# Skylarking/MARL

Hardware: AMD Instinct MI355X
Metric: env_steps_per_sec (higher is better)
Workload: dtype f32 (bf16x6 split products, fp32 accumulate)

## Files before the change

include/marl_hip.h:

```cpp
#ifndef MARL_HIP_H
#define MARL_HIP_H
#include <stddef.h>
#ifdef __cplusplus
extern "C" {
#endif

typedef struct {
  const float* p0; long ld0; int k0;
  const float* p1; long ld1; int k1;
  const int* idx; int nhot; int hot_w;
  int nid;
  const float* m0; long ldm0;
  long rpe0, bs0, off0;
  long rpei, bsi, offi;
  const int* emap0;
} marl_src_t;

typedef struct {
  int groups;
  long gs_x0, gs_x1, gs_w, gs_b, gs_y, gs_m0;
} marl_group_t;

typedef struct {
  const float *fc1_w, *fc1_b;
// ... 86 lines not shown
int marl_qmix_wide_fwd(const marl_qmix_weights_t* w, const marl_src_t* s, const float* q, float* q_tot, float* ws,
                       size_t ws_bytes, long rows, int N, int S, int E, int flags, void* stream);
int marl_qmix_wide_bwd(const marl_qmix_weights_t* w, const marl_src_t* s, const float* q, const float* dq_tot, float* dq,
                       const marl_qmix_weights_t* grads, float* ws, size_t ws_bytes, long rows, int N, int S, int E,
                       int flags, void* stream);
int marl_qmix_wide_loss_bwd(const marl_qmix_weights_t* w, const marl_src_t* s, const float* q, const float* q_tot_tgt,
                            const float* r, const float* term, const float* padded, float gamma, float* q_tot, float* dq,
                            const marl_qmix_weights_t* grads, float* loss2, float* ws, size_t ws_bytes, long rows,
                            int N, int S, int E, int flags, void* stream);

typedef struct {
  const float *w1, *b1;
  const float *w2, *b2;
  const float *w3, *b3;
  long gs_w1, gs_b1, gs_w2, gs_b2, gs_w3, gs_b3;
} marl_mlp3_weights_t;
int marl_mlp3_supported(const marl_src_t* x, int K1, int H1, int H2, int N3, int groups);
int marl_mlp3_fwd(const marl_mlp3_weights_t* w, const marl_src_t* x, float* Y, long ldy, long gs_y,
                  long M, int K1, int N3, int groups, void* stream);
size_t marl_mlp3_bwd_workspace(long M, int K1, int N3, int groups);
int marl_mlp3_bwd(const marl_mlp3_weights_t* w, const marl_src_t* x, const float* dY, long lddy, long gs_dy,
                  const marl_mlp3_weights_t* grads, float* ws, size_t ws_bytes, long M, int K1, int N3,
                  int groups, void* stream);
size_t marl_mlp3_save_floats(long M, int three, int groups);
int marl_mlp3_needs_kept(const marl_src_t* x, int K1, int N3);
int marl_mlp3_fwd_save(const marl_mlp3_weights_t* w, const marl_src_t* x, float* Y, long ldy, long gs_y,
                       float* hsave, size_t hsave_floats, long M, int K1, int N3, int groups, void* stream);
int marl_mlp3_bwd_saved(const marl_mlp3_weights_t* w, const marl_src_t* x, const float* dY, long lddy, long gs_dy,
                        const marl_mlp3_weights_t* grads, float* ws, size_t ws_bytes, const float* hsave,
                        size_t hsave_floats, long M, int K1, int N3, int groups, void* stream);

int marl_agent_unroll_x6_supported(int B, int T, int N, int O, int A, int last_action, int reuse_network);
int marl_agent_unroll_x6_plain_r6(int B, int T, int N, int O, int A, int last_action, int reuse_network, int cu_budget);
int marl_agent_unroll_fwd_x6(const marl_agent_weights_t* w, const float* obs, long obs_bs, int obs_t0,
                             const int* ufed, long u_bs, int u_t0, const int* ep_len, const int* ep_map,
                             const float* h0, float* q, float* hs, float* h_last, float* saved, int B, int T, int N,
                             int O, int A, int last_action, int reuse_network, int cu_budget, float* gi_out,
                             const float* gi_in, void* stream);

int marl_agent_unroll_bwd_x6_supported(int B, int T, int N, int A, int sparse_dq);
size_t marl_agent_bwd_x6_workspace(int B, int N, int A);
int marl_agent_unroll_bwd_x6(const marl_agent_weights_t* w, const int* dq_idx, const float* dq_val, const int* dq_idx2,
                             const float* dq_val2, int dq_gdiv, const float* dhs, const float* saved, float* dxp, float* dh0,
                             const marl_agent_grads_t* g, float* ws, size_t ws_bytes, int B, int T, int N, int A, void* stream);

int marl_mlp3_x6_supported(const marl_src_t* x, int K1, int H1, int H2, int N3, int groups);
int marl_mlp3_x6_fwd_save(const marl_mlp3_weights_t* w, const marl_src_t* x, float* Y, long ldy, long gs_y,
                          float* hsave, size_t hsave_floats, long M, int K1, int N3, int groups, void* stream);
int marl_mlp3_x6_bwd_saved(const marl_mlp3_weights_t* w, const marl_src_t* x, const float* dY, long lddy, long gs_dy,
                           const marl_mlp3_weights_t* grads, float* ws, size_t ws_bytes, const float* hsave,
                           size_t hsave_floats, long M, int K1, int N3, int groups, void* stream);

typedef struct {
  const float *enc0_w, *enc0_b;
  const float *enc2_w, *enc2_b;
  const float* q0_w; long q0_ld; int q0_s;
  const float *q2_w, *q2_b;
  const float *q4_w, *q4_b;
} marl_qtran_weights_t;
int marl_qtran_supported(int N, int A, int AE);
int marl_qtran_head_fwd(const marl_qtran_weights_t* w, const float* hidden, const int* u, const float* sp, float* out,
                        float* s1, float* e2, float* y1, float* y2, long BT, int N, int A, int AE, void* stream);
int marl_qtran_head_fwd2(const marl_qtran_weights_t* w, const float* hidden, const int* u, const int* u2, const float* sp,
                         float* out, float* out2, float* s1, float* e2, float* y1, float* y2, long BT, int N, int A, int AE,
                         void* stream);
size_t marl_qtran_bwd_workspace(long BT, int AE);
// ... 143 lines not shown
```

marl_amd/_lib.py:

```python
from __future__ import annotations

import ctypes as C
import os

_HERE = os.path.dirname(os.path.abspath(__file__))
LIB_PATH = os.environ.get("MARL_HIP_LIB") or os.path.join(_HERE, "libmarl_hip.so")

c_float_p = C.c_void_p
c_int_p = C.c_void_p


class MarlSrc(C.Structure):
    _fields_ = [("p0", C.c_void_p), ("ld0", C.c_long), ("k0", C.c_int),
                ("p1", C.c_void_p), ("ld1", C.c_long), ("k1", C.c_int),
                ("idx", C.c_void_p), ("nhot", C.c_int), ("hot_w", C.c_int),
                ("nid", C.c_int),
                ("m0", C.c_void_p), ("ldm0", C.c_long),
                ("rpe0", C.c_long), ("bs0", C.c_long), ("off0", C.c_long),
                ("rpei", C.c_long), ("bsi", C.c_long), ("offi", C.c_long),
                ("emap0", C.c_void_p)]


class MarlGroup(C.Structure):
    _fields_ = [("groups", C.c_int), ("gs_x0", C.c_long), ("gs_x1", C.c_long), ("gs_w", C.c_long),
# ... 38 lines not shown
                                          "k_w", "k_b", "q_w", "q_b")]


class MarlAgentGrads(C.Structure):
    _fields_ = [("w_ih", C.c_void_p), ("w_hh", C.c_void_p), ("b_ih", C.c_void_p), ("b_hh", C.c_void_p),
                ("fc2_w", C.c_void_p), ("fc2_b", C.c_void_p)]


class MarlAgentWeights(C.Structure):
    _fields_ = [("fc1_w", C.c_void_p), ("fc1_b", C.c_void_p), ("w_ih", C.c_void_p), ("w_hh", C.c_void_p),
                ("b_ih", C.c_void_p), ("b_hh", C.c_void_p), ("fc2_w", C.c_void_p), ("fc2_b", C.c_void_p),
                ("H", C.c_int)]


P, I, L, F, U, SZ, D = C.c_void_p, C.c_int, C.c_long, C.c_float, C.c_uint, C.c_size_t, C.c_double
SRC, GRP, AW = C.POINTER(MarlSrc), C.POINTER(MarlGroup), C.POINTER(MarlAgentWeights)
AG = C.POINTER(MarlAgentGrads)
QW = C.POINTER(MarlQmixWeights)
M3 = C.POINTER(MarlMlp3Weights)
QT = C.POINTER(MarlQtranWeights)
RW = C.POINTER(MarlRtwWeights)
WW, WG = C.POINTER(MarlWorldWeights), C.POINTER(MarlWorldGrads)
MW, MG = C.POINTER(MarlMaicWeights), C.POINTER(MarlMaicGrads)

SIGNATURES = {
    "marl_linear": (I, [SRC, P, L, I, P, P, L, I, I, I, I, F, GRP, P]),
    "marl_linear_wgrad": (I, [P, L, P, L, SRC, P, L, P, I, I, I, I, GRP, P, SZ, P]),
    "marl_linear_wgrad_workspace": (SZ, [I, I, I, I]),
    "marl_wgrad_slabs": (I, [I]),
    "marl_agent_unroll_fwd": (I, [AW, P, L, I, P, L, I, P, P, P, P, P, P, P, I, I, I, I, I, I, I, I, P, P, P]),
    "marl_agent_unroll_reuse_supported": (I, [I, I, I, I, I, I]),
    "marl_agent_unroll_x6_supported": (I, [I, I, I, I, I, I, I]),
    "marl_agent_unroll_x6_plain_r6": (I, [I, I, I, I, I, I, I, I]),
    "marl_agent_unroll_fwd_x6": (I, [AW, P, L, I, P, L, I, P, P, P, P, P, P, P, I, I, I, I, I, I, I, I, P, P, P]),
    "marl_agent_bwd_workspace": (SZ, [I, I, I]),
    "marl_agent_unroll_bwd_x6_supported": (I, [I, I, I, I, I]),
    "marl_agent_bwd_x6_workspace": (SZ, [I, I, I]),
    "marl_agent_unroll_bwd_x6": (I, [AW, P, P, P, P, I, P, P, P, P, AG, P, SZ, I, I, I, I, P]),
    "marl_agent_unroll_bwd": (I, [AW, P, P, P, P, P, I, P, P, P, P, P, AG, P, SZ, I, I, I, I, P]),
    "marl_replay_gather": (I, [P, I, I, I, I] + [P] * 17 + [P]),
    "marl_q_gather": (I, [P, P, P, F, P, L, I, P]),
    "marl_q_masked_max": (I, [P, P, F, P, P, L, I, P]),
    "marl_q_double_select": (I, [P, P, P, F, P, P, L, I, P]),
    "marl_q_scatter": (I, [P, P, P, P, P, L, I, I, P]),
    "marl_vec_add": (I, [P, P, P, L, P]),
    "marl_agent_sum": (I, [P, L, P, L, L, I, I, P]),
    "marl_agent_bcast": (I, [P, L, P, L, L, I, I, I, P]),
    "marl_qmix_mix_fwd": (I, [P, L, P, P, P, P, P, L, I, I, P]),
    "marl_qmix_mix_bwd": (I, [P, L, P, P, P, P, P, P, L, I, I, P]),
    "marl_qmix_tail_fwd": (I, [SRC, L, I, P, L, P, P, L, P, P, L, I, I, P]),
    "marl_qmix_fused_supported": (I, [I, I, I]),
    "marl_qmix_fused_workspace": (SZ, [L, I, I]),
    "marl_qmix_fused_fwd": (I, [QW, SRC, P, P, L, I, I, I, P]),
    "marl_qmix_fused_bwd": (I, [QW, SRC, P, P, P, QW, P, SZ, L, I, I, I, P]),
    "marl_qmix_fused_loss_bwd": (I, [QW, SRC, P, P, P, P, P, F, P, P, QW, P, P, SZ, L, I, I, I, P]),
    "marl_qmix_fused_fwd_x6": (I, [QW, SRC, P, P, L, I, I, I, P]),
    "marl_qmix_fused_bwd_x6": (I, [QW, SRC, P, P, P, QW, P, SZ, L, I, I, I, P]),
    "marl_qmix_fused_loss_bwd_x6": (I, [QW, SRC, P, P, P, P, P, F, P, P, QW, P, P, SZ, L, I, I, I, P]),
    "marl_qmix_wide_supported": (I, [I, I, I]),
    "marl_qmix_wide_workspace": (SZ, [L, I, I, I]),
    "marl_qmix_wide_fwd_kernel": (C.c_char_p, [L, I, I, I]),
    "marl_qmix_wide_fwd": (I, [QW, SRC, P, P, P, SZ, L, I, I, I, I, P]),
    "marl_qmix_wide_bwd": (I, [QW, SRC, P, P, P, QW, P, SZ, L, I, I, I, I, P]),
    "marl_qmix_wide_loss_bwd": (I, [QW, SRC, P, P, P, P, P, F, P, P, QW, P, P, SZ, L, I, I, I, I, P]),
    "marl_mlp3_supported": (I, [SRC, I, I, I, I, I]),
    "marl_mlp3_fwd": (I, [M3, SRC, P, L, L, L, I, I, I, P]),
# ... 89 lines not shown
```

marl_amd/csrc/agent_x6.hip:

```cpp
#include "x6.h"
#include <cstdlib>
#include "../../include/marl_hip.h"

int marl_agent_x6p_tiles(int B, int T, int N, int O, int A, int last_action, int reuse_network, int cu_budget);
int marl_agent_x6p_launch(const marl_agent_weights_t* w, const float* obs, long obs_bs, int obs_t0, const int* ufed, long u_bs, int u_t0,
                          const int* ep_len, const int* ep_map, const float* h0, float* q, float* h_last, int B, int T, int N, int O, int A,
                          int last_action, int reuse_network, int tpw, void* stream);

namespace {

constexpr int H = 64;
constexpr int XNT = 512;
constexpr int HP = 72;
constexpr int NLD = 4;

struct X6Args {
  const float *W1, *b1, *Wih, *Whh, *bih, *bhh, *W2, *b2;
  const float* obs; long obs_bs; int obs_t0;
  const int* ufed; long u_bs; int u_t0;
  const int* ep_len; const int* ep_map;
  const float* h0;
  float *q, *hs, *h_last;
  float* saved;
  float* gi_out;
  const float* gi_in;
  int B, T, N, O, A, I, KI;
  int has_act, has_id, RT;
  int n_full;
  long R;
};

__device__ __forceinline__ f32x4 relu4x(const f32x4& v) { return (f32x4){fmaxf(v[0], 0.f), fmaxf(v[1], 0.f), fmaxf(v[2], 0.f), fmaxf(v[3], 0.f)}; }
__device__ __forceinline__ long sv_off(long tile_t, int planes, int plane, int c, int lane) {
  return ((tile_t * planes + plane) * 4 + c) * 256 + lane * 4;
}

template <int RTC, bool SAVE, bool XS, bool GIO = false, int NK1 = 3, int AC = 1>
__global__ __launch_bounds__(XNT, 2) void agent_fwd_x6_kernel(X6Args a) {
  static_assert(!(SAVE && XS) && (SAVE || !GIO), "XS: no saving; GIO: the saving pass also stores its input-side gate sums");
  extern __shared__ __attribute__((aligned(16))) char smem[];
// ... 384 lines not shown
        }
      }
      if (!FC2I && t > 0 && s < RTW) fc2(par, t - 1, s);
      if (NGR && t + 1 < a.T) nin(par ^ 1, t + 1);
      ST_MARK(2);
      if (ALLP) {
        if (par) commit(0, pu_lds0); else commit(1, pu_lds1);
        issue(t + 4 < a.T ? t + 4 : Tm1);
      }
      WG_BARRIER();
      ST_MARK(3);
    }
    if (!FC2I && s < RTW) fc2(a.T & 1, a.T - 1, s);
    ST_DUMP(4);
  }
}

}

extern "C" int marl_agent_unroll_x6_supported(int B, int T, int N, int O, int A, int last_action, int reuse_network) {
  const int I = O + (last_action ? A : 0) + (reuse_network ? N : 0);
  if (A < 1 || O < 8 || (O & 7) || I > 224 || T < 4 || B < 1) return 0;
  if (A > (I > 160 ? 32 : 16)) return 0;
  if (16 * (O / 4) > 3 * 256) return 0;
  if ((double)B * T * N * H * 4.0 >= 4294967296.0) return 0;
  return 1;
}

extern "C" int marl_agent_unroll_x6_plain_r6(int B, int T, int N, int O, int A, int last_action, int reuse_network, int cu_budget) {
  return marl_agent_unroll_x6_supported(B, T, N, O, A, last_action, reuse_network) &&
         marl_agent_x6p_tiles(B, T, N, O, A, last_action, reuse_network, cu_budget) ? 1 : 0;
}

extern "C" int marl_agent_unroll_fwd_x6(const marl_agent_weights_t* w, const float* obs, long obs_bs, int obs_t0,
                                        const int* ufed, long u_bs, int u_t0, const int* ep_len, const int* ep_map,
                                        const float* h0, float* q, float* hs, float* h_last, float* saved, int B, int T, int N,
                                        int O, int A, int last_action, int reuse_network, int cu_budget, float* gi_out,
                                        const float* gi_in, void* stream) {
  if (B <= 0 || T <= 0) return 0;
  if (w->H != H || cu_budget < 0 || cu_budget > 256 || !marl_agent_unroll_x6_supported(B, T, N, O, A, last_action, reuse_network))
    return (int)hipErrorInvalidValue;
  if (saved && gi_in) return (int)hipErrorInvalidValue;
  if (!saved && !gi_in && !hs && !(reinterpret_cast<uintptr_t>(h0) & 15) && !(reinterpret_cast<uintptr_t>(h_last) & 15)) {
    const int tpw = marl_agent_x6p_tiles(B, T, N, O, A, last_action, reuse_network, cu_budget);
    if (tpw) return marl_agent_x6p_launch(w, obs, obs_bs, obs_t0, ufed, u_bs, u_t0, ep_len, ep_map, h0, q, h_last, B, T, N, O, A, last_action,
                                          reuse_network, tpw, stream);
  }
  if ((reinterpret_cast<uintptr_t>(obs) & 15) || (h0 && (reinterpret_cast<uintptr_t>(h0) & 3)) || (saved && (reinterpret_cast<uintptr_t>(saved) & 15)) ||
      (gi_out && (reinterpret_cast<uintptr_t>(gi_out) & 15)) || (gi_in && (reinterpret_cast<uintptr_t>(gi_in) & 15)))
    return (int)hipErrorInvalidValue;
  if (cu_budget == 0) cu_budget = 256;
  X6Args a;
  a.W1 = w->fc1_w; a.b1 = w->fc1_b; a.Wih = w->w_ih; a.Whh = w->w_hh; a.bih = w->b_ih; a.bhh = w->b_hh; a.W2 = w->fc2_w; a.b2 = w->fc2_b;
  a.obs = obs; a.obs_bs = obs_bs; a.obs_t0 = obs_t0; a.ufed = ufed; a.u_bs = u_bs; a.u_t0 = u_t0; a.ep_len = ep_len; a.ep_map = ep_map;
  a.h0 = h0; a.q = q; a.hs = hs; a.h_last = h_last; a.saved = saved; a.gi_out = saved ? gi_out : nullptr; a.gi_in = gi_in;
  a.B = B; a.T = T; a.N = N; a.O = O; a.A = A;
  a.has_act = last_action ? 1 : 0; a.has_id = reuse_network ? 1 : 0;
  a.I = O + (last_action ? A : 0) + (reuse_network ? N : 0);
  a.KI = (a.I + 31) / 32 * 32;
  a.R = (long)B * N;
  const long tiles = (a.R + 15) / 16;
  const int wide = a.KI > 160 ? 2 : a.KI > 96 ? 1 : 0;
  const int rt = tiles > cu_budget && !wide ? 2 : 1;
  if (rt * 16 * (O / 4) > 3 * 256) return (int)hipErrorInvalidValue;
  a.RT = rt;
  long n_wg = (tiles + rt - 1) / rt;
  a.n_full = (int)n_wg;
  if (rt == 2) {
    const long k = (tiles + 2 * cu_budget - 1) / (2 * cu_budget), rem = tiles - 2L * cu_budget * (k - 1);
    if (rem <= cu_budget) { a.n_full = (int)(cu_budget * (k - 1)); n_wg = a.n_full + rem; }
  }
  const int rows = rt * 16, IP = a.KI + 8;
  const size_t lds = (size_t)2 * 3 * rows * IP * 2 + (size_t)4 * 3 * rows * HP * 2 + (size_t)2 * rt * 4 * 3 * 1024 + (size_t)rows * (2 * 8 + 4 * 4) +
                     (((size_t)T * 4 + 15) & ~(size_t)15) + (wide == 2 ? (size_t)4 * 2 * 3 * 1024 : 0);
  if (lds > 160 * 1024) return (int)hipErrorInvalidValue;
  const void* fn;
#define X6_PICKF(SAVE_, XS_, GIO_) (wide == 2 ? (const void*)agent_fwd_x6_kernel<1, SAVE_, XS_, GIO_, 7, 2>                         \
                                    : wide == 1 ? (const void*)agent_fwd_x6_kernel<1, SAVE_, XS_, GIO_, 5, 1>                       \
                                    : rt == 2 ? (const void*)agent_fwd_x6_kernel<2, SAVE_, XS_, GIO_, 3, 1> : (const void*)agent_fwd_x6_kernel<1, SAVE_, XS_, GIO_, 3, 1>)
// ... 17 lines not shown
```

marl_amd/csrc/agent_x6p.hip:

```cpp
#include "x6.h"
#include "../../include/marl_hip.h"

namespace {

constexpr int H = 64;
constexpr int PNT = 512;
constexpr int HP = 72;
constexpr int NPF = 7;

struct PX6Args {
  const float *W1, *b1, *Wih, *Whh, *bih, *bhh, *W2, *b2;
  const float* obs; long obs_bs; int obs_t0;
  const int* ufed; long u_bs; int u_t0;
  const int* ep_len; const int* ep_map;
  const float* h0;
  float *q, *h_last;
  int B, T, N, O, A, I, KI;
  int has_act, has_id;
  long R;
};

template <int RTC>
__global__ __launch_bounds__(PNT, 2) void agent_fwd_x6p_kernel(PX6Args a) {
  extern __shared__ __attribute__((aligned(16))) char smem[];
  const int tid = threadIdx.x, lane = tid & 63, wave = __builtin_amdgcn_readfirstlane(tid >> 6);
  const int team = wave >> 2, s = wave & 3;
  const int q = lane >> 4, m = lane & 15, u4 = 16 * s + 4 * q;
  constexpr int rows = 16 * RTC;
  const int T = a.T, N = a.N, O = a.O, A = a.A;
  const int IP = a.KI + 8;
  const int IN_E = 3 * rows * IP, XP_E = 3 * rows * HP;
  short* In0 = reinterpret_cast<short*>(smem);
  short* Xp0 = In0 + IN_E;
  short* Hp0 = Xp0 + XP_E;
  float* W1a = reinterpret_cast<float*>(Hp0 + 2 * XP_E);
  unsigned* rowobs = reinterpret_cast<unsigned*>(W1a + (A + 1) * H);
  unsigned* rowu = rowobs + rows;
  int* rowidx = reinterpret_cast<int*>(rowu + rows);
  int* rowlen = rowidx + rows;
  i32x4* W2f = reinterpret_cast<i32x4*>(rowlen + rows);
  auto hpp = [&](int b) { return Hp0 + b * XP_E; };

  const long row0 = (long)blockIdx.x * rows;
  for (int r = tid; r < rows; r += PNT) {
    long rho = row0 + r;
    if (rho > a.R - 1) rho = a.R - 1;
    const long b = rho / N;
    const int n = (int)(rho % N);
    rowidx[r] = (int)(b * T * N + n);
    rowobs[r] = (unsigned)((((a.ep_map ? (long)a.ep_map[b] : b) * a.obs_bs + n) * O) * 4);
    rowu[r] = (unsigned)((b * a.u_bs + n) * 4);
    rowlen[r] = a.ep_len ? a.ep_len[b] : 0x7fffffff;
// ... 245 lines not shown
    };
    issue(0);
    ufetch(0);
    commit(0);
    WG_BARRIER();
    fc1();
    xput(0);
    issue(1); ufetch(1);
    WG_BARRIER();
    commit(1);
    issue(2);
    WG_BARRIER();
    ST_DECL(4);
    for (int t = 0; t < T; ++t) {
      if (t + 1 < T) fc1();
      if (t >= 1) fc2(t & 1, t - 1, true);
      else landed();
      ST_MARK(0);
      WG_BARRIER();
      ST_MARK(1);
      if (t + 1 < T) xput(t + 1);
      commit(t + 2);
      issue(t + 3);
      ufetch(t + 2);
      ST_MARK(2);
      WG_BARRIER();
      ST_MARK(3);
    }
    ST_DUMP(4);
    fc2(T & 1, T - 1, false);
  }
}

static size_t px6_lds(int rtc, int KI, int A) {
  const size_t rows = 16 * (size_t)rtc, IP = KI + 8;
  return 3 * rows * IP * 2 + 3 * 3 * rows * HP * 2 + (size_t)(A + 1) * H * 4 + rows * (4 + 4 + 4 + 4) + (rtc >= 5 ? (size_t)2 * 3 * 4 * A * 16 : 0);
}

}

ST_DEFINE_SETTER(marl_debug_stamps_agent_x6p)

__attribute__((visibility("hidden"))) int marl_agent_x6p_tiles(int B, int T, int N, int O, int A, int last_action, int reuse_network, int cu_budget) {
  if (!marl_switches()->unroll_r6) return 0;
  const int I = O + (last_action ? A : 0) + (reuse_network ? N : 0);
  if (I > 96 || A < 1 || A > 16 || O < 8 || (O & 3) || T < 2 || B < 1) return 0;
  if (cu_budget != 0 && cu_budget != 256) return 0;
  const long tiles = ((long)B * N + 15) / 16;
  if (tiles <= 512) return 0;
  if ((long)16 * 5 * (O / 4) > 256L * NPF) return 0;
  if (T > 32000) return 0;
  if ((double)B * T * N * H * 4.0 >= 4294967296.0) return 0;
  int tpw = (int)((tiles + 255) / 256);
  if (tpw > 5) {
    const long rounds = (tiles + 256 * 5 - 1) / (256 * 5);
    tpw = (int)((tiles + 256 * rounds - 1) / (256 * rounds));
    if (tpw > 5) tpw = 5;
  }
  if (tpw < 3) tpw = 3;
  return px6_lds(tpw, (I + 31) / 32 * 32, A) <= 160 * 1024 ? tpw : 0;
}

__attribute__((visibility("hidden"))) int marl_agent_x6p_launch(const marl_agent_weights_t* w, const float* obs, long obs_bs, int obs_t0,
                                                                 const int* ufed, long u_bs, int u_t0, const int* ep_len, const int* ep_map,
                                                                 const float* h0, float* q, float* h_last, int B, int T, int N, int O, int A,
                                                                 int last_action, int reuse_network, int tpw, void* stream) {
  if ((reinterpret_cast<uintptr_t>(obs) & 15) || (h0 && (reinterpret_cast<uintptr_t>(h0) & 15)) || (h_last && (reinterpret_cast<uintptr_t>(h_last) & 15)))
    return (int)hipErrorInvalidValue;
  PX6Args a;
  a.W1 = w->fc1_w; a.b1 = w->fc1_b; a.Wih = w->w_ih; a.Whh = w->w_hh; a.bih = w->b_ih; a.bhh = w->b_hh; a.W2 = w->fc2_w; a.b2 = w->fc2_b;
  a.obs = obs; a.obs_bs = obs_bs; a.obs_t0 = obs_t0; a.ufed = ufed; a.u_bs = u_bs; a.u_t0 = u_t0; a.ep_len = ep_len; a.ep_map = ep_map;
  a.h0 = h0; a.q = q; a.h_last = h_last;
  a.B = B; a.T = T; a.N = N; a.O = O; a.A = A;
  a.has_act = last_action ? 1 : 0; a.has_id = reuse_network ? 1 : 0;
  a.I = O + (last_action ? A : 0) + (reuse_network ? N : 0);
  a.KI = (a.I + 31) / 32 * 32;
  a.R = (long)B * N;
  const long tiles = (a.R + 15) / 16;
  const size_t lds = px6_lds(tpw, a.KI, A);
  const void* fn = tpw == 3 ? (const void*)agent_fwd_x6p_kernel<3> : tpw == 4 ? (const void*)agent_fwd_x6p_kernel<4> : (const void*)agent_fwd_x6p_kernel<5>;
  hipError_t e = hipFuncSetAttribute(fn, hipFuncAttributeMaxDynamicSharedMemorySize, (int)lds);
  if (e != hipSuccess) return (int)e;
  dim3 grid((unsigned)((tiles + tpw - 1) / tpw)), block(PNT);
  void* kargs[] = {(void*)&a};
  e = hipLaunchKernel(fn, grid, block, kargs, lds, (hipStream_t)stream);
  if (e != hipSuccess) return (int)e;
  MARL_CHECK_LAUNCH();
  return 0;
}
```

marl_amd/ops.py:

```python
from __future__ import annotations

import ctypes as C

import torch

from . import _lib
from ._lib import (MarlSrc, MarlGroup, MarlAgentWeights, MarlAgentGrads, MarlQmixWeights, MarlMlp3Weights,
                   MarlQtranWeights, MarlRtwWeights, MarlWorldWeights, MarlWorldGrads, MarlMaicWeights, MarlMaicGrads, check)


def _p(t):
    return None if t is None else C.c_void_p(t.data_ptr())


def _stream():
    return C.c_void_p(torch.cuda.current_stream().cuda_stream)


def _f32(t):
    assert t.dtype == torch.float32 and t.is_cuda, "expected a CUDA float32 tensor"
    return t


def _i32(t):
# ... 105 lines not shown
    w = MarlAgentWeights()
    w.fc1_w, w.fc1_b = params["fc1.weight"].data_ptr(), params["fc1.bias"].data_ptr()
    w.w_ih, w.w_hh = params["rnn.weight_ih"].data_ptr(), params["rnn.weight_hh"].data_ptr()
    w.b_ih, w.b_hh = params["rnn.bias_ih"].data_ptr(), params["rnn.bias_hh"].data_ptr()
    w.fc2_w, w.fc2_b = params["fc2.weight"].data_ptr(), params["fc2.bias"].data_ptr()
    w.H = params["rnn.weight_hh"].shape[1]
    for k in ("fc1.weight", "rnn.weight_ih", "rnn.weight_hh", "fc2.weight"):
        assert params[k].is_contiguous() and params[k].dtype == torch.float32 and params[k].is_cuda
    w._keep = params
    return w


def agent_unroll_fwd(w, obs, obs_bs, obs_t0, ufed, u_bs, u_t0, h0, q, hs, h_last, saved,
                     B, T, N, O, A, last_action=True, reuse_network=True, ep_len=None, ep_map=None, cu_budget=0, gi_out=None,
                     gi_in=None):
    lib = _lib.load()
    check(lib.marl_agent_unroll_fwd(C.byref(w), _p(_f32(obs)), obs_bs, obs_t0, _p(ufed), u_bs, u_t0, _p(ep_len),
                                    _p(_i32(ep_map)) if ep_map is not None else None, _p(h0),
                                    _p(_f32(q)), _p(hs), _p(h_last), _p(saved), B, T, N, O, A,
                                    1 if last_action else 0, 1 if reuse_network else 0, int(cu_budget),
                                    _p(_f32(gi_out)) if gi_out is not None else None,
                                    _p(_f32(gi_in)) if gi_in is not None else None, _stream()),
          "marl_agent_unroll_fwd")


def agent_unroll_x6_supported(B, T, N, O, A, last_action=True, reuse_network=True):
    return bool(_lib.load().marl_agent_unroll_x6_supported(B, T, N, O, A, 1 if last_action else 0, 1 if reuse_network else 0))


def agent_unroll_x6_plain_r6(B, T, N, O, A, last_action=True, reuse_network=True, cu_budget=0):
    return bool(_lib.load().marl_agent_unroll_x6_plain_r6(B, T, N, O, A, 1 if last_action else 0, 1 if reuse_network else 0, int(cu_budget)))


def agent_unroll_fwd_x6(w, obs, obs_bs, obs_t0, ufed, u_bs, u_t0, h0, q, hs, h_last, saved, B, T, N, O, A, last_action=True,
                        reuse_network=True, ep_len=None, ep_map=None, cu_budget=0, gi_out=None, gi_in=None):
    if saved is None and gi_in is None and hs is None and agent_unroll_x6_plain_r6(B, T, N, O, A, last_action, reuse_network, cu_budget):
        assert obs.numel() < 2 ** 30 and (ufed is None or ufed.numel() < 2 ** 30), "observation storage beyond 4 GB: set MARL_UNROLL_R6=0"
    check(_lib.load().marl_agent_unroll_fwd_x6(C.byref(w), _p(_f32(obs)), obs_bs, obs_t0, _p(ufed), u_bs, u_t0, _p(ep_len),
                                               _p(_i32(ep_map)) if ep_map is not None else None, _p(h0), _p(_f32(q)), _p(hs),
                                               _p(h_last), _p(saved), B, T, N, O, A, 1 if last_action else 0,
                                               1 if reuse_network else 0, int(cu_budget),
                                               _p(_f32(gi_out)) if gi_out is not None else None,
                                               _p(_f32(gi_in)) if gi_in is not None else None, _stream()),
          "marl_agent_unroll_fwd_x6")


def saved_shape(T, B, N, planes=6, H=64):
    return (T + (1 if planes == 6 else 0), (B * N + 15) // 16 * 16, planes, H)


def saved_plane(saved, plane, rows):
    T, R16, P, H = saved.shape
    t = saved.reshape(T, R16 // 16, P, 4, 4, 16, 4)[:, :, plane]
    return t.permute(0, 1, 3, 5, 2, 4).reshape(T, R16, H)[:, :rows]


def agent_unroll_reuse_supported(B, T, N, O, A, cu_budget=0):
    return bool(_lib.load().marl_agent_unroll_reuse_supported(B, T, N, O, A, int(cu_budget)))


def agent_unroll_bwd_x6_supported(B, T, N, A, sparse_dq=True):
    return bool(_lib.load().marl_agent_unroll_bwd_x6_supported(B, T, N, A, 1 if sparse_dq else 0))


def agent_unroll_bwd(w, dq, dhs, saved, hs, dxp, dh0, grads, B, T, N, A, dq_idx=None, dq_val=None, dq_idx2=None,
                     dq_val2=None, dq_gdiv=1, x6=False):
    lib = _lib.load()
    g = MarlAgentGrads()
    g.w_ih, g.w_hh = grads["rnn.weight_ih"].data_ptr(), grads["rnn.weight_hh"].data_ptr()
# ... 601 lines not shown
```

Measured before the change: 73.87 million.

## Add persistent R6 agent forward kernel that consumes precomputed gi_in

Adds an xs variant of the persistent register-resident agent forward kernel, used when gi_in (precomputed input-gate activations) is supplied. Previously any call with gi_in fell back to the generic path. One team of waves runs the GRU recurrence and streams gi_in through LDS with double-buffered prefetch, while the other team computes fc2 outputs, and fc1/input gates only at masked steps. Routing logic moves into a new route function that checks alignment, 32-bit offset limits and LDS fit. This adds a large new kernel and more LDS use, which may reduce occupancy.

```diff
diff --git a/include/marl_hip.h b/include/marl_hip.h
--- a/include/marl_hip.h
+++ b/include/marl_hip.h
@@ -142,6 +142,8 @@
 
 int marl_agent_unroll_x6_supported(int B, int T, int N, int O, int A, int last_action, int reuse_network);
 int marl_agent_unroll_x6_plain_r6(int B, int T, int N, int O, int A, int last_action, int reuse_network, int cu_budget);
+int marl_agent_unroll_x6_r6_tiles(int B, int T, int N, int O, int A, int last_action, int reuse_network, int cu_budget, long obs_bs,
+                                  long u_bs, int has_ep_map, const void* h0, const void* h_last, int xs);
 int marl_agent_unroll_fwd_x6(const marl_agent_weights_t* w, const float* obs, long obs_bs, int obs_t0,
                              const int* ufed, long u_bs, int u_t0, const int* ep_len, const int* ep_map,
                              const float* h0, float* q, float* hs, float* h_last, float* saved, int B, int T, int N,
diff --git a/marl_amd/_lib.py b/marl_amd/_lib.py
--- a/marl_amd/_lib.py
+++ b/marl_amd/_lib.py
@@ -94,6 +94,7 @@
     "marl_agent_unroll_reuse_supported": (I, [I, I, I, I, I, I]),
     "marl_agent_unroll_x6_supported": (I, [I, I, I, I, I, I, I]),
     "marl_agent_unroll_x6_plain_r6": (I, [I, I, I, I, I, I, I, I]),
+    "marl_agent_unroll_x6_r6_tiles": (I, [I, I, I, I, I, I, I, I, L, L, I, P, P, I]),
     "marl_agent_unroll_fwd_x6": (I, [AW, P, L, I, P, L, I, P, P, P, P, P, P, P, I, I, I, I, I, I, I, I, P, P, P]),
     "marl_agent_bwd_workspace": (SZ, [I, I, I]),
     "marl_agent_unroll_bwd_x6_supported": (I, [I, I, I, I, I]),
diff --git a/marl_amd/csrc/agent_x6.hip b/marl_amd/csrc/agent_x6.hip
--- a/marl_amd/csrc/agent_x6.hip
+++ b/marl_amd/csrc/agent_x6.hip
@@ -3,9 +3,11 @@
 #include "../../include/marl_hip.h"
 
 int marl_agent_x6p_tiles(int B, int T, int N, int O, int A, int last_action, int reuse_network, int cu_budget);
+int marl_agent_x6p_route(int B, int T, int N, int O, int A, int last_action, int reuse_network, int cu_budget, long obs_bs, long u_bs,
+                         int has_map, const void* h0, const void* h_last, int xs);
 int marl_agent_x6p_launch(const marl_agent_weights_t* w, const float* obs, long obs_bs, int obs_t0, const int* ufed, long u_bs, int u_t0,
                           const int* ep_len, const int* ep_map, const float* h0, float* q, float* h_last, int B, int T, int N, int O, int A,
-                          int last_action, int reuse_network, int tpw, void* stream);
+                          int last_action, int reuse_network, int tpw, const float* gi_in, void* stream);
 
 namespace {
 
@@ -456,6 +458,12 @@
          marl_agent_x6p_tiles(B, T, N, O, A, last_action, reuse_network, cu_budget) ? 1 : 0;
 }
 
+extern "C" int marl_agent_unroll_x6_r6_tiles(int B, int T, int N, int O, int A, int last_action, int reuse_network, int cu_budget, long obs_bs,
+                                             long u_bs, int has_ep_map, const void* h0, const void* h_last, int xs) {
+  if (!marl_agent_unroll_x6_supported(B, T, N, O, A, last_action, reuse_network)) return 0;
+  return marl_agent_x6p_route(B, T, N, O, A, last_action, reuse_network, cu_budget, obs_bs, u_bs, has_ep_map, h0, h_last, xs);
+}
+
 extern "C" int marl_agent_unroll_fwd_x6(const marl_agent_weights_t* w, const float* obs, long obs_bs, int obs_t0,
                                         const int* ufed, long u_bs, int u_t0, const int* ep_len, const int* ep_map,
                                         const float* h0, float* q, float* hs, float* h_last, float* saved, int B, int T, int N,
@@ -465,10 +473,10 @@
   if (w->H != H || cu_budget < 0 || cu_budget > 256 || !marl_agent_unroll_x6_supported(B, T, N, O, A, last_action, reuse_network))
     return (int)hipErrorInvalidValue;
   if (saved && gi_in) return (int)hipErrorInvalidValue;
-  if (!saved && !gi_in && !hs && !(reinterpret_cast<uintptr_t>(h0) & 15) && !(reinterpret_cast<uintptr_t>(h_last) & 15)) {
-    const int tpw = marl_agent_x6p_tiles(B, T, N, O, A, last_action, reuse_network, cu_budget);
+  if (!saved && !hs && !(gi_in && (reinterpret_cast<uintptr_t>(gi_in) & 15))) {
+    const int tpw = marl_agent_x6p_route(B, T, N, O, A, last_action, reuse_network, cu_budget, obs_bs, u_bs, ep_map ? 1 : 0, h0, h_last, gi_in ? 1 : 0);
     if (tpw) return marl_agent_x6p_launch(w, obs, obs_bs, obs_t0, ufed, u_bs, u_t0, ep_len, ep_map, h0, q, h_last, B, T, N, O, A, last_action,
-                                          reuse_network, tpw, stream);
+                                          reuse_network, tpw, gi_in, stream);
   }
   if ((reinterpret_cast<uintptr_t>(obs) & 15) || (h0 && (reinterpret_cast<uintptr_t>(h0) & 3)) || (saved && (reinterpret_cast<uintptr_t>(saved) & 15)) ||
       (gi_out && (reinterpret_cast<uintptr_t>(gi_out) & 15)) || (gi_in && (reinterpret_cast<uintptr_t>(gi_in) & 15)))
diff --git a/marl_amd/csrc/agent_x6p.hip b/marl_amd/csrc/agent_x6p.hip
--- a/marl_amd/csrc/agent_x6p.hip
+++ b/marl_amd/csrc/agent_x6p.hip
@@ -18,6 +18,7 @@
   int B, T, N, O, A, I, KI;
   int has_act, has_id;
   long R;
+  const float* gi_in;
 };
 
 template <int RTC>
@@ -329,6 +330,252 @@
   }
 }
 
+constexpr int GSP = 4 * 68;
+constexpr int GSS = 3 * GSP;
+
+template <int RTC>
+__global__ __launch_bounds__(PNT, 2) void agent_fwd_x6p_xs_kernel(PX6Args a) {
+  extern __shared__ __attribute__((aligned(16))) char smem[];
+  const int tid = threadIdx.x, lane = tid & 63, wave = __builtin_amdgcn_readfirstlane(tid >> 6);
+  const int team = wave >> 2, s = wave & 3;
+  const int q = lane >> 4, m = lane & 15, u4 = 16 * s + 4 * q, u = 16 * s + m;
+  constexpr int rows = 16 * RTC;
+  const int T = a.T, N = a.N, O = a.O, A = a.A;
+  const int IP = a.KI + 8;
+  const int XP_E = 3 * rows * HP;
+  float* GI0 = reinterpret_cast<float*>(smem);
+  short* Hp0 = reinterpret_cast<short*>(GI0 + RTC * 4 * GSS);
+  short* In1 = Hp0 + 2 * XP_E;
+  short* Xp1 = In1 + 3 * 16 * IP;
+  unsigned* rowobs = reinterpret_cast<unsigned*>(Xp1 + 3 * 16 * HP);
+  unsigned* rowu = rowobs + rows;
+  int* rowidx = reinterpret_cast<int*>(rowu + rows);
+  int* rowlen = rowidx + rows;
+  int* rown = rowlen + rows;
+  int* xmask = rown + rows;
+  auto hpp = [&](int b) { return Hp0 + b * XP_E; };
+
+  const long NTILES = (a.R + 15) >> 4;
+  const long tile0 = (long)blockIdx.x * RTC, row0 = tile0 * 16;
+  for (int r = tid; r < rows; r += PNT) {
+    long rho = row0 + r;
+    if (rho > a.R - 1) rho = a.R - 1;
+    const long b = rho / N;
+    const int n = (int)(rho % N);
+    rowidx[r] = (int)(b * T * N + n);
+    rowobs[r] = (unsigned)((((a.ep_map ? (long)a.ep_map[b] : b) * a.obs_bs + n) * O) * 4);
+    rowu[r] = (unsigned)((b * a.u_bs + n) * 4);
+    rowlen[r] = a.ep_len ? a.ep_len[b] : 0x7fffffff;
+    rown[r] = n;
+  }
+  for (int e = tid; e < T; e += PNT) xmask[e] = e == T - 1 ? 1 : 0;
+  for (int e = tid; e < (3 * 16 * IP + 3 * 16 * HP) / 2; e += PNT) reinterpret_cast<int*>(In1)[e] = 0;
+  __syncthreads();
+  if (tid < rows) { const int L = rowlen[tid]; if (L >= 1 && L - 1 < T) xmask[L - 1] = 1; }
+  const int Tm1 = T - 1;
+  const int KC1 = a.KI >> 5;
+
+  if (team == 0) {
+    F3 wh[6];
+#pragma unroll
+    for (int g = 0; g < 3; ++g)
+#pragma unroll
+      for (int c = 0; c < 2; ++c) wh[2 * g + c] = wfrag(a.Whh, H, g * H + 16 * s, 3 * H, H, c, lane);
+    f32x4 bias_hn;
+#pragma unroll
+    for (int r = 0; r < 4; ++r) bias_hn[r] = a.bhh[2 * H + u4 + r];
+    f32x4 hreg[RTC];
+#pragma unroll
+    for (int rt = 0; rt < RTC; ++rt) {
+      long rho = row0 + rt * 16 + m; if (rho > a.R - 1) rho = a.R - 1;
+      hreg[rt] = a.h0 ? *reinterpret_cast<const f32x4*>(a.h0 + rho * H + u4) : splat(0.f);
+      put4t(hpp(0), HP, rows * HP, rt * 16 + m, u4, hreg[rt]);
+    }
+    unsigned gof[RTC];
+#pragma unroll
+    for (int rt = 0; rt < RTC; ++rt) {
+      const long tl = tile0 + rt < NTILES ? tile0 + rt : NTILES - 1;
+      gof[rt] = (unsigned)(tl * 12288 + s * 1024 + lane * 16);
+    }
+    f32x4 gB[RTC][3];
+    auto gload = [&](int t, int rt) __attribute__((always_inline)) {
+      const char* gb = reinterpret_cast<const char*>(a.gi_in + (long)(t < Tm1 ? t + 1 : Tm1) * NTILES * 3072);
+#pragma unroll
+      for (int k = 0; k < 3; ++k) gB[rt][k] = *reinterpret_cast<const f32x4*>(gb + (size_t)(gof[rt] + 4096u * k));
+    };
+    float* const gsw = GI0 + s * GSS + q * 68 + m * 4;
+    const float* const gsr = GI0 + s * GSS + (m >> 2) * 68 + 16 * q + (m & 3);
+    auto gput = [&](int rt) __attribute__((always_inline)) {
+#pragma unroll
+      for (int k = 0; k < 3; ++k) *reinterpret_cast<f32x4*>(gsw + rt * 4 * GSS + k * GSP) = gB[rt][k];
+    };
+    auto gget = [&](int rt, f32x4 (&g)[3]) __attribute__((always_inline)) {
+#pragma unroll
+      for (int k = 0; k < 3; ++k)
+#pragma unroll
+        for (int j = 0; j < 4; ++j) g[k][j] = gsr[rt * 4 * GSS + k * GSP + 4 * j];
+    };
+#pragma unroll
+    for (int rt = 0; rt < RTC; ++rt) gload(0, rt);
+#pragma unroll
+    for (int rt = 0; rt < RTC; ++rt) { gput(rt); gload(1, rt); }
+    WG_BARRIER();
+    ST_DECL(4);
+    for (int t = 0; t < T; ++t) {
+      const int par = t & 1;
+      if (__builtin_amdgcn_readfirstlane(xmask[t])) {
+        for (int i = 0; i < 2 * RTC + 1; ++i) WG_BARRIER();
+      }
+      f32x4 G[2][4], gn[3];
+      gget(0, gn);
+#pragma unroll
+      for (int rt = 0; rt <= RTC; ++rt) {
+        if (rt < RTC) {
+          f32x4* g = G[rt & 1];
+          g[0] = gn[0]; g[1] = gn[1]; g[2] = gn[2]; g[3] = bias_hn;
+          gput(rt);
+          gload(t + 2, rt);
+          if (rt + 1 < RTC) gget(rt + 1, gn);
+          const F3 fc = bfrag(hpp(par) + rt * 16 * HP, HP, rows * HP, 0, lane);
+          const F3 fd = bfrag(hpp(par) + rt * 16 * HP, HP, rows * HP, 1, lane);
+#define OP(p_, q_) g[0] = mm(wh[0].q_, fc.p_, g[0]); g[1] = mm(wh[2].q_, fc.p_, g[1]); g[3] = mm(wh[4].q_, fc.p_, g[3]);
+          X6_TERMS(OP)
+#undef OP
+#define OP(p_, q_) g[0] = mm(wh[1].q_, fd.p_, g[0]); g[1] = mm(wh[3].q_, fd.p_, g[1]); g[3] = mm(wh[5].q_, fd.p_, g[3]);
+          X6_TERMS(OP)
+#undef OP
+        }
+        if (rt > 0) {
+          const f32x4* g = G[(rt - 1) & 1];
+          f32x4 hn;
+#pragma unroll
+          for (int r = 0; r < 4; ++r) hn[r] = gru_h_x6(g[0][r], g[1][r], g[2][r], g[3][r], hreg[rt - 1][r]);
+          put4t(hpp(par ^ 1), HP, rows * HP, (rt - 1) * 16 + m, u4, hn);
+          hreg[rt - 1] = hn;
+        }
+        if (rt > 0 && rt < RTC) {
+#pragma unroll
+          for (int i = 0; i < 36; ++i) {
+            __builtin_amdgcn_sched_group_barrier(0x008, 1, 0);
+            __builtin_amdgcn_sched_group_barrier(0x002, 1, 0);
+          }
+        }
+      }
+      ST_MARK(0);
+      WG_BARRIER();
+      ST_MARK(1);
+    }
+    ST_DUMP(4);
+    if (a.h_last) {
+#pragma unroll
+      for (int rt = 0; rt < RTC; ++rt) {
+        const long rho = row0 + rt * 16 + m;
+        if (rho < a.R) *reinterpret_cast<f32x4*>(a.h_last + rho * H + u4) = hreg[rt];
+      }
+    }
+  } else {
+    const int ti = tid - PNT / 2;
+    F3 w1[3], wi[6], w2[2];
+#pragma unroll
+    for (int c = 0; c < 3; ++c) w1[c] = c < KC1 ? wfrag(a.W1, a.I, 16 * s, H, a.I, c, lane) : F3{};
+#pragma unroll
+    for (int g = 0; g < 3; ++g)
+#pragma unroll
+      for (int c = 0; c < 2; ++c) wi[2 * g + c] = wfrag(a.Wih, H, g * H + 16 * s, 3 * H, H, c, lane);
+#pragma unroll
+    for (int c = 0; c < 2; ++c) w2[c] = wfrag(a.W2, H, 0, A, H, c, lane);
+    const float bias_1 = a.b1[u], bias_r = a.bih[u] + a.bhh[u], bias_z = a.bih[H + u] + a.bhh[H + u], bias_n = a.bih[2 * H + u];
+    const float bias_2 = m < A ? a.b2[m] : 0.f;
+    const int O4 = O >> 2, CW = a.KI - O;
+    auto intile = [&](int t, int rt) __attribute__((always_inline)) {
+      const char* ob = reinterpret_cast<const char*>(a.obs + (long)(t + a.obs_t0) * N * O);
+      for (int e = ti; e < 16 * O4; e += PNT / 2) {
+        const int r = e / O4, k4 = e - r * O4, rr = rt * 16 + r;
+        f32x4 v = *reinterpret_cast<const f32x4*>(ob + (size_t)(rowobs[rr] + 16u * (unsigned)k4));
+        if (!(t < rowlen[rr])) v = splat(0.f);
+        const F3h f = split4(v);
+        short* p = In1 + r * IP + 4 * k4;
+        *reinterpret_cast<i32x2*>(p) = f.h;
+        *reinterpret_cast<i32x2*>(p + 16 * IP) = f.m;
+        *reinterpret_cast<i32x2*>(p + 2 * 16 * IP) = f.l;
+      }
+      const bool fed = a.has_act && a.ufed && t + a.u_t0 >= 0;
+      const char* ub = reinterpret_cast<const char*>(a.ufed + (fed ? (long)(t + a.u_t0) * N : 0));
+      for (int e = ti; e < 16 * CW; e += PNT / 2) {
+        const int r = e / CW, k = O + (e - r * CW), rr = rt * 16 + r;
+        const int uu = fed ? *reinterpret_cast<const int*>(ub + (size_t)rowu[rr]) : -1;
+        const bool one = (a.has_act && uu >= 0 && uu < A && k - O == uu) || (a.has_id && k >= a.I - N && k < a.I && rown[rr] == k - (a.I - N));
+        In1[r * IP + k] = one ? (short)0x3F80 : (short)0;
+        In1[16 * IP + r * IP + k] = 0;
+        In1[2 * 16 * IP + r * IP + k] = 0;
+      }
+    };
+    auto fc1 = [&]() __attribute__((always_inline)) {
+      f32x4 acc[3] = {splat(bias_1), splat(0.f), splat(0.f)};
+#pragma unroll
+      for (int c = 0; c < 3; ++c) mm6(bfrag(In1, IP, 16 * IP, c < KC1 ? c : 0, lane), w1[c], acc[c]);
+      const f32x4 v = (acc[0] + acc[1]) + acc[2];
+      const f32x4 x = {fmaxf(v[0], 0.f), fmaxf(v[1], 0.f), fmaxf(v[2], 0.f), fmaxf(v[3], 0.f)};
+      put4(Xp1, HP, 16 * HP, 4 * q, u, x);
+    };
+    auto gih = [&](int rt) __attribute__((always_inline)) {
+      f32x4 ag[3] = {splat(bias_r), splat(bias_z), splat(bias_n)};
+#pragma unroll
+      for (int c = 0; c < 2; ++c) {
+        const F3 xb = bfrag(Xp1, HP, 16 * HP, c, lane);
+#define OP(p_, q_) _Pragma("unroll") for (int g = 0; g < 3; ++g) ag[g] = mm(xb.p_, wi[2 * g + c].q_, ag[g]);
+        X6_TERMS(OP)
+#undef OP
+      }
+      float* gp = GI0 + (rt * 4 + s) * GSS + q * 68 + m * 4;
+#pragma unroll
+      for (int k = 0; k < 3; ++k) *reinterpret_cast<f32x4*>(gp + k * GSP) = ag[k];
+    };
+    constexpr int QT = (RTC + 3) / 4;
+    auto fc2 = [&](int bh, int ts) __attribute__((always_inline)) {
+#pragma unroll
+      for (int k = 0; k < QT; ++k) {
+        const int rt = 4 * k + s;
+        if (rt < RTC && tile0 + rt < NTILES) {
+          F3 hb[2];
+#pragma unroll
+          for (int c = 0; c < 2; ++c) hb[c] = bfrag(hpp(bh) + rt * 16 * HP, HP, rows * HP, c, lane);
+          f32x4 ac[2] = {splat(bias_2), splat(0.f)};
+#define OP(p_, q_) _Pragma("unroll") for (int c = 0; c < 2; ++c) ac[c] = mm(hb[c].p_, w2[c].q_, ac[c]);
+          X6_TERMS(OP)
+#undef OP
+          const f32x4 qa = ac[0] + ac[1];
+          if (m < A) {
+#pragma unroll
+            for (int r = 0; r < 4; ++r) a.q[(unsigned)(rowidx[rt * 16 + 4 * q + r] + ts * N) * (unsigned)A + (unsigned)m] = qa[r];
+          }
+        }
+      }
+    };
+    WG_BARRIER();
+    ST_DECL(4);
+    for (int t = 0; t < T; ++t) {
+      if (__builtin_amdgcn_readfirstlane(xmask[t])) {
+#pragma unroll 1
+        for (int rt = 0; rt < RTC; ++rt) {
+          intile(t, rt);
+          WG_BARRIER();
+          fc1();
+          WG_BARRIER();
+          gih(rt);
+        }
+        WG_BARRIER();
+      }
+      if (t >= 1) fc2(t & 1, t - 1);
+      ST_MARK(0);
+      WG_BARRIER();
+      ST_MARK(1);
+    }
+    ST_DUMP(4);
+    fc2(T & 1, T - 1);
+  }
+}
+
 static size_t px6_lds(int rtc, int KI, int A) {
   const size_t rows = 16 * (size_t)rtc, IP = KI + 8;
   return 3 * rows * IP * 2 + 3 * 3 * rows * HP * 2 + (size_t)(A + 1) * H * 4 + rows * (4 + 4 + 4 + 4) + (rtc >= 5 ? (size_t)2 * 3 * 4 * A * 16 : 0);
@@ -358,11 +605,33 @@
   return px6_lds(tpw, (I + 31) / 32 * 32, A) <= 160 * 1024 ? tpw : 0;
 }
 
+static size_t px6xs_lds(int rtc, int KI, int T) {
+  const size_t rows = 16 * (size_t)rtc, IP = KI + 8;
+  return (size_t)rtc * 4 * GSS * 4 + 2 * 3 * rows * HP * 2 + 3 * 16 * IP * 2 + 3 * 16 * HP * 2 + rows * 5 * 4 + (((size_t)T * 4 + 15) & ~(size_t)15);
+}
+
+__attribute__((visibility("hidden"))) int marl_agent_x6p_route(int B, int T, int N, int O, int A, int last_action, int reuse_network, int cu_budget,
+                                                                long obs_bs, long u_bs, int has_map, const void* h0, const void* h_last, int xs) {
+  const int tpw = marl_agent_x6p_tiles(B, T, N, O, A, last_action, reuse_network, cu_budget);
+  if (!tpw) return 0;
+  if ((reinterpret_cast<uintptr_t>(h0) & 15) || (reinterpret_cast<uintptr_t>(h_last) & 15)) return 0;
+  if (!has_map && (((double)B * (double)obs_bs + N) * O * 4.0 >= 4294967296.0 || (double)B * (double)u_bs * 4.0 >= 4294967296.0)) return 0;
+  if (obs_bs < 0 || u_bs < 0) return 0;
+  if (xs) {
+    const int I = O + (last_action ? A : 0) + (reuse_network ? N : 0);
+    const long tiles = ((long)B * N + 15) / 16;
+    if ((double)tiles * 12288.0 >= 4294967296.0) return 0;
+    if (px6xs_lds(tpw, (I + 31) / 32 * 32, T) > 160 * 1024) return 0;
+  }
+  return tpw;
+}
+
 __attribute__((visibility("hidden"))) int marl_agent_x6p_launch(const marl_agent_weights_t* w, const float* obs, long obs_bs, int obs_t0,
                                                                  const int* ufed, long u_bs, int u_t0, const int* ep_len, const int* ep_map,
                                                                  const float* h0, float* q, float* h_last, int B, int T, int N, int O, int A,
-                                                                 int last_action, int reuse_network, int tpw, void* stream) {
-  if ((reinterpret_cast<uintptr_t>(obs) & 15) || (h0 && (reinterpret_cast<uintptr_t>(h0) & 15)) || (h_last && (reinterpret_cast<uintptr_t>(h_last) & 15)))
+                                                                 int last_action, int reuse_network, int tpw, const float* gi_in, void* stream) {
+  if ((reinterpret_cast<uintptr_t>(obs) & 15) || (h0 && (reinterpret_cast<uintptr_t>(h0) & 15)) || (h_last && (reinterpret_cast<uintptr_t>(h_last) & 15)) ||
+      (reinterpret_cast<uintptr_t>(gi_in) & 15))
     return (int)hipErrorInvalidValue;
   PX6Args a;
   a.W1 = w->fc1_w; a.b1 = w->fc1_b; a.Wih = w->w_ih; a.Whh = w->w_hh; a.bih = w->b_ih; a.bhh = w->b_hh; a.W2 = w->fc2_w; a.b2 = w->fc2_b;
@@ -373,9 +642,11 @@
   a.I = O + (last_action ? A : 0) + (reuse_network ? N : 0);
   a.KI = (a.I + 31) / 32 * 32;
   a.R = (long)B * N;
+  a.gi_in = gi_in;
   const long tiles = (a.R + 15) / 16;
-  const size_t lds = px6_lds(tpw, a.KI, A);
-  const void* fn = tpw == 3 ? (const void*)agent_fwd_x6p_kernel<3> : tpw == 4 ? (const void*)agent_fwd_x6p_kernel<4> : (const void*)agent_fwd_x6p_kernel<5>;
+  const size_t lds = gi_in ? px6xs_lds(tpw, a.KI, T) : px6_lds(tpw, a.KI, A);
+  const void* fn = gi_in ? (tpw == 3 ? (const void*)agent_fwd_x6p_xs_kernel<3> : tpw == 4 ? (const void*)agent_fwd_x6p_xs_kernel<4> : (const void*)agent_fwd_x6p_xs_kernel<5>)
+                         : (tpw == 3 ? (const void*)agent_fwd_x6p_kernel<3> : tpw == 4 ? (const void*)agent_fwd_x6p_kernel<4> : (const void*)agent_fwd_x6p_kernel<5>);
   hipError_t e = hipFuncSetAttribute(fn, hipFuncAttributeMaxDynamicSharedMemorySize, (int)lds);
   if (e != hipSuccess) return (int)e;
   dim3 grid((unsigned)((tiles + tpw - 1) / tpw)), block(PNT);
diff --git a/marl_amd/ops.py b/marl_amd/ops.py
--- a/marl_amd/ops.py
+++ b/marl_amd/ops.py
@@ -161,9 +161,17 @@
     return bool(_lib.load().marl_agent_unroll_x6_plain_r6(B, T, N, O, A, 1 if last_action else 0, 1 if reuse_network else 0, int(cu_budget)))
 
 
+def agent_unroll_x6_r6_tiles(B, T, N, O, A, last_action=True, reuse_network=True, cu_budget=0, obs_bs=0, u_bs=0, ep_map=False, h0=0,
+                             h_last=0, xs=False):
+    ad = lambda t: C.c_void_p(int(t.data_ptr()) if hasattr(t, "data_ptr") else int(t or 0))
+    return int(_lib.load().marl_agent_unroll_x6_r6_tiles(B, T, N, O, A, 1 if last_action else 0, 1 if reuse_network else 0, int(cu_budget),
+                                                         int(obs_bs), int(u_bs), 1 if ep_map else 0, ad(h0), ad(h_last), 1 if xs else 0))
+
+
 def agent_unroll_fwd_x6(w, obs, obs_bs, obs_t0, ufed, u_bs, u_t0, h0, q, hs, h_last, saved, B, T, N, O, A, last_action=True,
                         reuse_network=True, ep_len=None, ep_map=None, cu_budget=0, gi_out=None, gi_in=None):
-    if saved is None and gi_in is None and hs is None and agent_unroll_x6_plain_r6(B, T, N, O, A, last_action, reuse_network, cu_budget):
+    if saved is None and hs is None and ep_map is not None and agent_unroll_x6_r6_tiles(
+            B, T, N, O, A, last_action, reuse_network, cu_budget, obs_bs, u_bs, True, h0, h_last, gi_in is not None):
         assert obs.numel() < 2 ** 30 and (ufed is None or ufed.numel() < 2 ** 30), "observation storage beyond 4 GB: set MARL_UNROLL_R6=0"
     check(_lib.load().marl_agent_unroll_fwd_x6(C.byref(w), _p(_f32(obs)), obs_bs, obs_t0, _p(ufed), u_bs, u_t0, _p(ep_len),
                                                _p(_i32(ep_map)) if ep_map is not None else None, _p(h0), _p(_f32(q)), _p(hs),
```

New measurement: 70.69 million. 4.3% lower.
